# Dahan-Wang/Rethinking-Flow-and-Diffusion-Bridge-Models-for-Speech-Enhancement

Hardware: NVIDIA B200
Metric: enhanced audio-sec/sec (5-step SB bridge, ncsnpp_v2) (higher is better)
Workload: dtype fp16

## Files before the change

rethinking-flow-and-diffusion-bridge-models-for-speech-enhancement_b200/csrc/conv_igemm.cu:

```cuda
#include <cuda.h>
#include <mutex>
#include <type_traits>
#include "common.cuh"
#include "tc05.cuh"

namespace fdbm {
int make_act_tile_map(CUtensorMap* map, const op_t* ptr, int B, int T, int F, int C, int box_f, int box_t);
namespace {

using namespace tc05;

constexpr int MT = 2;
constexpr int TILE_T = 16, TILE_F = 8;
constexpr int HALO_T = TILE_T + 2, HALO_F = TILE_F + 2;
constexpr int A_TILE_BYTES = HALO_T * HALO_F * 128;
constexpr int A_TILE_STRIDE = 23552;
constexpr int A_STAGES = 3;
constexpr int B_STAGES = 3;
constexpr int BN = 128;
constexpr int B_TILE_BYTES = BN * 128;
constexpr int A_SBO = HALO_F * 128;
constexpr int NUM_THREADS = 512;
constexpr int EPI_GROUPS = 2;
constexpr int MAX_SEG = 3;
// ... 58 lines not shown

template <typename F>
__device__ __forceinline__ void walk_steps(const ConvParams& p, F&& f) {
  const int n_side = p.n_kb - p.n_main;
  int sd = 0, cnt = 0;
  for (int m = 0; m < p.n_main; ++m) {
    const int ntaps = p.seg[p.ksched[m] & 15].taps;
    for (int tap = 0; tap < ntaps; ++tap) {
      f(false, m, tap, ntaps);
      if (++cnt == p.side_gap && sd < n_side) { f(true, p.n_main + sd, 0, 1); ++sd; cnt = 0; }
    }
  }
  for (; sd < n_side; ++sd) f(true, p.n_main + sd, 0, 1);
}

template <bool COMB, bool RES16>
__global__ void __launch_bounds__(NUM_THREADS, 1)
conv_igemm_kernel(const __grid_constant__ CUtensorMap map_a0, const __grid_constant__ CUtensorMap map_a1,
                  const __grid_constant__ CUtensorMap map_a2, const __grid_constant__ CUtensorMap map_b,
                  const ConvParams p) {
  extern __shared__ __align__(1024) uint8_t smem_raw[];
  uint8_t* smem = smem_raw;
  if (smem_u32(smem_raw) & 1023u) __trap();
  uint8_t* sA = smem;
  uint8_t* sB = smem + A_STAGES * MT * A_TILE_STRIDE;
  uint8_t* s_stage = sB + B_STAGES * B_TILE_BYTES;
  uint8_t* s_stat = s_stage + STAGE_BYTES;
  uint64_t* bars = reinterpret_cast<uint64_t*>(s_stage + STAGE_BYTES + STAT_BYTES);
  uint64_t* a_full = bars;
  uint64_t* a_empty = a_full + A_STAGES;
  uint64_t* b_full = a_empty + A_STAGES;
  uint64_t* b_empty = b_full + B_STAGES_NARROW;
  uint64_t* acc_full = b_empty + B_STAGES_NARROW;
  const int b_stages = p.bn == 16 ? B_STAGES_NARROW : B_STAGES;
  const int b_stride = p.bn * 128;
  uint64_t* acc_empty = acc_full + 2;
  uint64_t* a_ready = acc_empty + 2;
  uint64_t* side_full = a_ready + A_STAGES;
  uint64_t* side_empty = side_full + 1;
  uint32_t* tmem_slot = reinterpret_cast<uint32_t*>(side_empty + 1);
  static_assert((3 * A_STAGES + 2 * B_STAGES_NARROW + 4 + 2) * 8 + 4 <= 512, "barrier region");
  const int a_stages = p.side_ring ? A_STAGES - 1 : A_STAGES;
  const int n_main = p.side_ring ? p.n_main : p.n_kb;

  const int warp = __shfl_sync(0xffffffffu, static_cast<int>(threadIdx.x >> 5), 0), lane = threadIdx.x & 31;
  const int n_kb = p.n_kb;

  if (threadIdx.x == 0) {
    for (int i = 0; i < A_STAGES; ++i) { mbar_init(a_full + i, 1); mbar_init(a_empty + i, 1); mbar_init(a_ready + i, 128); }
    for (int i = 0; i < B_STAGES_NARROW; ++i) { mbar_init(b_full + i, 1); mbar_init(b_empty + i, 1); }
    for (int i = 0; i < 2; ++i) { mbar_init(acc_full + i, 1); mbar_init(acc_empty + i, 4 * EPI_GROUPS); }
    mbar_init(side_full, 1); mbar_init(side_empty, 1);
    fence_barrier_init();
  }
  if (warp == 0 && lane == 0) {
    tma_prefetch_desc(&map_a0);
    tma_prefetch_desc(&map_b);
    if (p.n_seg > 1) tma_prefetch_desc(&map_a1);
    if (p.n_seg > 2) tma_prefetch_desc(&map_a2);
  }
  if (warp == 3) {
    tmem_alloc(tmem_slot, 512);
    tmem_relinquish();
  }
  fence_before_sync();
  __syncthreads();
  fence_after_sync();
  const uint32_t tmem_base = *tmem_slot;
  asm volatile("griddepcontrol.wait;" ::: "memory");
  asm volatile("griddepcontrol.launch_dependents;" ::: "memory");

  if (warp < 4) {
  reg_dec<PIPE_REGS>();
  if (warp == 0) {
    if (lane == 0) {
      uint32_t stage = 0, phase = 0;
      for (int item = blockIdx.x; item < p.n_items; item += gridDim.x) {
        const int ct = item_tile(p, item);
        TileCoord tc[MT];
        int n_valid = 0;
        for (int j = 0; j < MT; ++j) { tc[j] = decode_tile(p, ct * MT + j); n_valid += tc[j].valid; }
        for (int i = 0; i < n_main; ++i) {
          const uint32_t e = p.ksched[i];
          const int sgi = e & 15, c0 = ((e >> 4) & 0xFFF) * 64;
          const int halo = p.seg[sgi].halo;
          mbar_wait_relaxed<256>(a_empty + stage, phase ^ 1);
          mbar_expect_tx(a_full + stage, n_valid * (halo ? A_TILE_BYTES : A_TILE1_BYTES));
          const CUtensorMap* map = sgi == 0 ? &map_a0 : (sgi == 1 ? &map_a1 : &map_a2);
          for (int j = 0; j < MT; ++j) {
            if (!tc[j].valid) continue;
            tma_load_4d(sA + (stage * MT + j) * A_TILE_STRIDE, map, a_full + stage, c0, tc[j].f0 - halo, tc[j].t0 - halo,
                        tc[j].b);
          }
          if (++stage == a_stages) { stage = 0; phase ^= 1; }
        }
      }
    }
  } else if (warp == 3) {
    if (lane == 0 && p.side_ring) {
      uint32_t phase = 0;
      for (int item = blockIdx.x; item < p.n_items; item += gridDim.x) {
        const int ct = item_tile(p, item);
        TileCoord tc[MT];
        int n_valid = 0;
        for (int j = 0; j < MT; ++j) { tc[j] = decode_tile(p, ct * MT + j); n_valid += tc[j].valid; }
        for (int i = n_main; i < n_kb; ++i) {
          const uint32_t e = p.ksched[i];
          const int sgi = e & 15, c0 = ((e >> 4) & 0xFFF) * 64;
          mbar_wait_relaxed<128>(side_empty, phase ^ 1);
          mbar_expect_tx(side_full, n_valid * A_TILE1_BYTES);
          const CUtensorMap* map = sgi == 0 ? &map_a0 : (sgi == 1 ? &map_a1 : &map_a2);
          for (int j = 0; j < MT; ++j) {
            if (!tc[j].valid) continue;
            tma_load_4d(sA + ((A_STAGES - 1) * MT + j) * A_TILE_STRIDE, map, side_full, c0, tc[j].f0, tc[j].t0, tc[j].b);
          }
          phase ^= 1;
        }
      }
    }
  } else if (warp == 1) {
    if (lane == 0) {
      uint32_t stage = 0, phase = 0;
      for (int item = blockIdx.x; item < p.n_items; item += gridDim.x) {
        const int n0 = item_nblk(p, item) * BN;
        if (p.side_ring) {
          walk_steps(p, [&](bool, int idx, int tap, int) {
            const int kt = static_cast<int>(p.ksched[idx] >> 16) + tap;
            mbar_wait_relaxed<128>(b_empty + stage, phase ^ 1);
            mbar_expect_tx(b_full + stage, b_stride);
            tma_load_2d(sB + stage * b_stride, &map_b, b_full + stage, 0, kt * p.Cout + n0);
            if (++stage == b_stages) { stage = 0; phase ^= 1; }
          });
          continue;
        }
        for (int i = 0; i < n_kb; ++i) {
          const uint32_t e = p.ksched[i];
          const int ntaps = p.seg[e & 15].taps;
          int kt = e >> 16;
          for (int tap = 0; tap < ntaps; ++tap, ++kt) {
            mbar_wait_relaxed<128>(b_empty + stage, phase ^ 1);
            mbar_expect_tx(b_full + stage, b_stride);
            tma_load_2d(sB + stage * b_stride, &map_b, b_full + stage, 0, kt * p.Cout + n0);
            if (++stage == b_stages) { stage = 0; phase ^= 1; }
          }
        }
      }
    }
  } else if (warp == 2) {
    const uint32_t idesc = make_idesc_f16(128, p.bn, kOperandIsBf16);
    const uint64_t a_hi9 = make_desc_sw128(0, A_SBO) & 0xFFFFFFFF00000000ull;
    const uint64_t a_hi1 = make_desc_sw128(0, TILE_F * 128) & 0xFFFFFFFF00000000ull;
    const uint64_t b_hi = make_desc_sw128(0, 1024) & 0xFFFFFFFF00000000ull;
    const uint32_t lo_const = 1u << 16;
    const uint32_t sA_lo = (smem_u32(sA) & 0x3FFFF) >> 4, sB_lo = (smem_u32(sB) & 0x3FFFF) >> 4;
    uint32_t sa = 0, pa = 0, sb = 0, pb = 0, as = 0, pacc = 0, ps = 0;
    for (int item = blockIdx.x; item < p.n_items; item += gridDim.x) {
      const int ct = item_tile(p, item);
      const bool valid1 = (ct * MT + 1) < p.n_mtiles;
      mbar_wait(acc_empty + as, pacc ^ 1);
      fence_after_sync();
      uint32_t accumulate = 0;
      const uint32_t d0 = tmem_base + (as * MT) * BN, d1 = d0 + BN;
      if (p.side_ring) {
        int step = 0;
        walk_steps(p, [&](bool side, int idx, int tap, int ntaps) {
          const SegParams& sg = p.seg[p.ksched[idx] & 15];
          uint32_t a_base0, a_off = 0;
          if (side) {
            mbar_wait(side_full, ps);
            fence_after_sync();
            a_base0 = sA_lo + (((A_STAGES - 1) * MT) * A_TILE_STRIDE >> 4);
          } else {
            if (tap == 0) {
// ... 1 lines not shown
              fence_after_sync();
            }
            a_base0 = sA_lo + ((sa * MT) * A_TILE_STRIDE >> 4);
            const int df = ntaps == 9 ? tap / 3 : sg.halo, dt = ntaps == 9 ? tap - 3 * (tap / 3) : sg.halo;
            a_off = ((dt * HALO_F + df) * 128) >> 4;
          }
          const uint64_t a_hi = sg.halo ? a_hi9 : a_hi1;
          mbar_wait(b_full + sb, pb);
          fence_after_sync();
          const uint32_t b_lo = (sB_lo + (sb * b_stride >> 4)) | lo_const;
          const uint32_t a_lo0 = (a_base0 + a_off) | lo_const, a_lo1 = (a_base0 + (A_TILE_STRIDE >> 4) + a_off) | lo_const;
          const bool last_tap = tap == ntaps - 1;
          if (elect_one()) {
#pragma unroll
            for (int k = 0; k < 4; ++k)
              mma_f16(d0, a_hi | (a_lo0 + 2 * k), b_hi | (b_lo + 2 * k), idesc, k == 0 ? accumulate : 1u);
            if (valid1) {
#pragma unroll
              for (int k = 0; k < 4; ++k)
                mma_f16(d1, a_hi | (a_lo1 + 2 * k), b_hi | (b_lo + 2 * k), idesc, k == 0 ? accumulate : 1u);
            }
            mma_commit(b_empty + sb);
            if (side) mma_commit(side_empty);
            else if (last_tap) mma_commit(a_empty + sa);
            if (step == p.n_steps - 1) mma_commit(acc_full + as);
          }
          __syncwarp();
          accumulate = 1;
          ++step;
          if (++sb == b_stages) { sb = 0; pb ^= 1; }
          if (side) ps ^= 1;
          else if (last_tap && ++sa == a_stages) { sa = 0; pa ^= 1; }
        });
        if (++as == 2) { as = 0; pacc ^= 1; }
        continue;
      }
      for (int i = 0; i < n_kb; ++i) {
        const SegParams& sg = p.seg[p.ksched[i] & 15];
        const int ntaps = sg.taps;
        const uint64_t a_hi = sg.halo ? a_hi9 : a_hi1;
        mbar_wait(sg.norm ? a_ready + sa : a_full + sa, pa);
        fence_after_sync();
        const uint32_t a_base0 = sA_lo + ((sa * MT) * A_TILE_STRIDE >> 4), a_base1 = a_base0 + (A_TILE_STRIDE >> 4);
        int df = ntaps == 9 ? 0 : sg.halo, dt = df;
        for (int tap = 0; tap < ntaps; ++tap) {
          mbar_wait(b_full + sb, pb);
          fence_after_sync();
          const uint32_t a_off = ((dt * HALO_F + df) * 128) >> 4;
          const uint32_t b_lo = (sB_lo + (sb * b_stride >> 4)) | lo_const;
          const uint32_t a_lo0 = (a_base0 + a_off) | lo_const, a_lo1 = (a_base1 + a_off) | lo_const;
          if (elect_one()) {
#pragma unroll
            for (int k = 0; k < 4; ++k)
              mma_f16(d0, a_hi | (a_lo0 + 2 * k), b_hi | (b_lo + 2 * k), idesc, k == 0 ? accumulate : 1u);
            if (valid1) {
#pragma unroll
              for (int k = 0; k < 4; ++k)
                mma_f16(d1, a_hi | (a_lo1 + 2 * k), b_hi | (b_lo + 2 * k), idesc, k == 0 ? accumulate : 1u);
            }
            mma_commit(b_empty + sb);
            if (tap == ntaps - 1) mma_commit(a_empty + sa);
            if (tap == ntaps - 1 && i == n_kb - 1) mma_commit(acc_full + as);
          }
          __syncwarp();
          accumulate = 1;
          if (++dt == 3) { dt = 0; ++df; }
          if (++sb == b_stages) { sb = 0; pb ^= 1; }
        }
        if (++sa == A_STAGES) { sa = 0; pa ^= 1; }
      }
      if (++as == 2) { as = 0; pacc ^= 1; }
    }
  }
  } else if (warp >= 8 && warp < 12) {
    reg_dec<XFORM_REGS>();
    const int tt = threadIdx.x - 256;
    const int g = tt & 7, p_lane = tt >> 3;
    uint32_t stage = 0, phase = 0;
    const bool any_norm = (p.seg[0].norm | p.seg[1].norm | p.seg[2].norm) != 0;
    for (int item = blockIdx.x; any_norm && item < p.n_items; item += gridDim.x) {
      const int ct = item_tile(p, item);
      TileCoord tc[MT];
      for (int j = 0; j < MT; ++j) tc[j] = decode_tile(p, ct * MT + j);
      for (int i = 0; i < n_main; ++i) {
        const uint32_t e = p.ksched[i];
        const SegParams& sg = p.seg[e & 15];
        float2 sc[MT][4], sh[MT][4];
        if (sg.norm) {
          const int c0 = ((e >> 4) & 0xFFF) * 64 + g * 8;
          const float pre = sg.act ? 0.5f : 1.0f;
#pragma unroll
          for (int j = 0; j < MT; ++j) {
            const float4* tp = reinterpret_cast<const float4*>(sg.tab + static_cast<int64_t>(tc[j].valid ? tc[j].b : 0) * sg.tab_stride + c0);
#pragma unroll
            for (int u = 0; u < 4; ++u) {
              const float4 e = __ldg(tp + u);
              sc[j][u] = make_float2(pre * e.x, pre * e.z); sh[j][u] = make_float2(pre * e.y, pre * e.w);
            }
// ... 56 lines not shown
                  slot[u] = reinterpret_cast<uint4*>(tile + px * 128 + ((g ^ (px & 7)) << 4));
                  raw[u] = on[u] ? *slot[u] : make_uint4(0u, 0u, 0u, 0u);
                }
#pragma unroll
                for (int u = 0; u < 4; ++u) xform(raw[u], act_tag);
#pragma unroll
                for (int u = 0; u < 4; ++u)
                  if (on[u]) *slot[u] = raw[u];
              }
            };
            if (interior) { if (sg.act) run_interior(std::true_type{}); else run_interior(std::false_type{}); }
            else { if (sg.act) run_border(std::true_type{}); else run_border(std::false_type{}); }
          }
          fence_proxy_async();
        }
        mbar_arrive(a_ready + stage);
        if (++stage == a_stages) { stage = 0; phase ^= 1; }
      }
    }
  } else {
    reg_inc<EPI_REGS>();
    const int q = warp & 3;
    const int eg = warp >= 12 ? 1 : 0;
    float4* stage = reinterpret_cast<float4*>(s_stage) + (eg * 4 + q) * (32 * 8);
    const int cc = lane & 7;
    const int rsub = lane >> 3;
    const int et = (threadIdx.x & 127);
    uint32_t as = 0, pacc = 0;
    const bool do_stats = p.sums != nullptr;
    float2* wstat = reinterpret_cast<float2*>(s_stat) + eg * 4 * BN;
    double acc_s[STAT_SLOTS], acc_q[STAT_SLOTS];
// ... 1 lines not shown
    for (int u = 0; u < STAT_SLOTS; ++u) { acc_s[u] = 0.0; acc_q[u] = 0.0; }
    int stat_b = -1;
    auto flush_stats = [&]() {
#pragma unroll
      for (int u = 0; u < STAT_SLOTS; ++u) {
        if (u < p.n_nblocks) {
          if (et < p.bn) {
            double* dst = p.sums + (static_cast<int64_t>(stat_b) * p.Cout + u * BN + et) * 2;
            atomicAdd(dst, acc_s[u]);
            atomicAdd(dst + 1, acc_q[u]);
          }
        }
        acc_s[u] = 0.0; acc_q[u] = 0.0;
      }
    };
    for (int item = blockIdx.x; item < p.n_items; item += gridDim.x) {
      const int ct = item_tile(p, item);
      const int nblk = item - ct * p.n_nblocks;
      const int n0 = nblk * BN;
      mbar_wait_relaxed(acc_full + as, pacc);
      fence_after_sync();
      for (int j = eg; j <= eg; ++j) {
        const TileCoord tc = decode_tile(p, ct * MT + j);
        if (!tc.valid) continue;
        if (do_stats && stat_b != tc.b) {
          if (stat_b >= 0) flush_stats();
          stat_b = tc.b;
        }
        if (p.pyr_out) {
          uint32_t v[32];
          tmem_ld_32x32(tmem_base + ((q * 32u) << 16) + (as * MT + j) * BN, v);
          tmem_ld_wait();
          const int m = q * 32 + lane;
          const int t = tc.t0 + (m >> 3), f = tc.f0 + (m & 7);
          if (t < p.T && f < p.F) {
            float o[4];
#pragma unroll
            for (int c = 0; c < 4; ++c) o[c] = c < p.pyr_C ? __uint_as_float(v[c]) + __ldg(p.bias + c) : 0.f;
// ... 212 lines not shown
          __syncwarp();
          bv = bvn; bvb = bvbn;
        }
        if (do_stats) {
          asm volatile("bar.sync %0, 128;" ::"r"(1 + eg) : "memory");
          double s = 0.0, sq = 0.0;
#pragma unroll
          for (int w = 0; w < 4; ++w) { const float2 e = et < p.bn ? wstat[w * BN + et] : make_float2(0.f, 0.f); s += e.x; sq += e.y; }
#pragma unroll
          for (int u = 0; u < STAT_SLOTS; ++u) if (u == nblk) { acc_s[u] += s; acc_q[u] += sq; }
          asm volatile("bar.sync %0, 128;" ::"r"(1 + eg) : "memory");
        }
      }
      fence_before_sync();
      __syncwarp();
      if (lane == 0) mbar_arrive(acc_empty + as);
      if (++as == 2) { as = 0; pacc ^= 1; }
    }
    if (do_stats && stat_b >= 0) flush_stats();
  }

  fence_before_sync();
  __syncthreads();
  if (warp == 3) tmem_dealloc(tmem_base, 512);
}

__device__ __forceinline__ void pack_fwd_element(const PackDesc& d, int64_t i) {
  const int C1 = d.C1, C2 = d.C2, Cout = d.Cout, ksize = d.ksize, io_layout = d.io;
  const int taps = ksize * ksize;
  const int j = static_cast<int>(i % 64);
  const int co = static_cast<int>((i / 64) % Cout);
  const int kt = static_cast<int>(i / (64ll * Cout));
  float v;
  if (io_layout == 2) {
    const int tap = j / C1, ci = j % C1;
    v = tap < 9 ? d.w1[((static_cast<int64_t>(co) * C1 + ci) * 3 + tap / 3) * 3 + tap % 3] : 0.f;
  } else if (kt < (C1 / 64) * taps) {
    const int kb = kt / taps, tap = kt % taps;
    const int ci = kb * 64 + j;
// ... 66 lines not shown

int make_weight_map(CUtensorMap* map, const op_t* ptr, int64_t rows, int bn) {
  EncodeFn enc = get_encode();
  if (!enc) { set_error("cuTensorMapEncodeTiled entry point not available"); return FDBM_ECUDA; }
  cuuint64_t dims[2] = {64, (cuuint64_t)rows};
  cuuint64_t strides[1] = {128};
  cuuint32_t box[2] = {64, (cuuint32_t)bn};
  cuuint32_t es[2] = {1, 1};
  CUresult r = enc(map, (kOperandIsBf16 ? CU_TENSOR_MAP_DATA_TYPE_BFLOAT16 : CU_TENSOR_MAP_DATA_TYPE_FLOAT16), 2, const_cast<op_t*>(ptr), dims, strides, box, es,
                   CU_TENSOR_MAP_INTERLEAVE_NONE, CU_TENSOR_MAP_SWIZZLE_128B, CU_TENSOR_MAP_L2_PROMOTION_L2_256B,
                   CU_TENSOR_MAP_FLOAT_OOB_FILL_NONE);
  if (r != CUDA_SUCCESS) { set_error("cuTensorMapEncodeTiled(weights, %lld rows) failed: %d", (long long)rows, (int)r); return FDBM_ECUDA; }
  return FDBM_OK;
}

}

int make_act_tile_map(CUtensorMap* map, const op_t* ptr, int B, int T, int F, int C, int box_f, int box_t) {
  EncodeFn enc = get_encode();
  if (!enc) { set_error("cuTensorMapEncodeTiled entry point not available"); return FDBM_ECUDA; }
  cuuint64_t dims[4] = {(cuuint64_t)C, (cuuint64_t)F, (cuuint64_t)T, (cuuint64_t)B};
  cuuint64_t strides[3] = {(cuuint64_t)C * 2, (cuuint64_t)C * 2 * F, (cuuint64_t)C * 2 * F * T};
  cuuint32_t box[4] = {64, (cuuint32_t)box_f, (cuuint32_t)box_t, 1};
  cuuint32_t es[4] = {1, 1, 1, 1};
  CUresult r = enc(map, (kOperandIsBf16 ? CU_TENSOR_MAP_DATA_TYPE_BFLOAT16 : CU_TENSOR_MAP_DATA_TYPE_FLOAT16), 4, const_cast<op_t*>(ptr), dims, strides, box, es,
                   CU_TENSOR_MAP_INTERLEAVE_NONE, CU_TENSOR_MAP_SWIZZLE_128B, CU_TENSOR_MAP_L2_PROMOTION_L2_256B,
                   CU_TENSOR_MAP_FLOAT_OOB_FILL_NONE);
  if (r != CUDA_SUCCESS) { set_error("cuTensorMapEncodeTiled(activation [%d,%d,%d,%d]) failed: %d", B, T, F, C, (int)r); return FDBM_ECUDA; }
  return FDBM_OK;
}
// ... 49 lines not shown
  const PackDesc d = pack_desc_dgrad(w, Cout, Cin, ksize, wpack, Cin_total, ci_off);
  pack_one_kernel<<<static_cast<int>(std::min<int64_t>(ceil_div64(d.total, 256), 4096)), 256, 0, s>>>(d);
  FDBM_LAUNCH_CHECK();
  return FDBM_OK;
}

int launch_conv_igemm(const ConvArgs& a, cudaStream_t s) {
  FDBM_REQUIRE(a.n_seg >= 1 && a.n_seg <= MAX_SEG, "conv_igemm: 1..%d K segments", MAX_SEG);
  const int bn = a.narrow_n ? 16 : (a.Cout == 64 ? 64 : BN);
  FDBM_REQUIRE(a.Cout % bn == 0 && (!a.narrow_n || (a.Cout == 16 && a.pyr_out)), "conv_igemm: Cout must be a multiple of %d (got %d)", bn, a.Cout);
  FDBM_REQUIRE(a.out_f32 || a.out_h16 || a.pyr_out, "conv_igemm: no output");
  FDBM_REQUIRE(!a.pyr_out || (a.pyr_C >= 1 && a.pyr_C <= 4 && a.Cout == bn && !a.sums), "conv_igemm: bad pyramid epilogue arguments");
  FDBM_REQUIRE(!a.pyr_prev || (a.T % 2 == 0 && a.F % 2 == 0), "conv_igemm: pyramid level with odd size");
  static PerDeviceOnce attr_once;
  if (attr_once.first(current_device())) {
    FDBM_CUDA(cudaFuncSetAttribute(conv_igemm_kernel<false, false>, cudaFuncAttributeMaxDynamicSharedMemorySize, SMEM_BYTES));
    FDBM_CUDA(cudaFuncSetAttribute(conv_igemm_kernel<false, true>, cudaFuncAttributeMaxDynamicSharedMemorySize, SMEM_BYTES));
    FDBM_CUDA(cudaFuncSetAttribute(conv_igemm_kernel<true, false>, cudaFuncAttributeMaxDynamicSharedMemorySize, SMEM_BYTES));
  }
  FDBM_REQUIRE(!a.comb_pyr || (a.comb_w && a.comb_b && a.comb_C >= 1 && a.comb_C <= 4 && !a.pyr_out), "conv_igemm: bad Combine epilogue arguments");
  CUtensorMap map_a[MAX_SEG], map_b;
  ConvParams p;
  p.B = a.B; p.T = a.T; p.F = a.F; p.Cout = a.Cout;
  p.n_seg = a.n_seg;
  int kb = 0, n_kt = 0;
  for (int i = 0; i < MAX_SEG; ++i) {
    if (i < a.n_seg) {
      const ConvSeg& sg = a.seg[i];
      FDBM_REQUIRE(sg.in && sg.C > 0 && sg.C % 64 == 0 && (sg.taps == 9 || sg.taps == 1),
                   "conv_igemm: segment %d needs a tensor, C %% 64 == 0 and 9 or 1 taps (C=%d, taps=%d)", i, sg.C, sg.taps);
      const int halo = sg.taps == 9 || sg.norm_tab != nullptr;
      if (int rc = halo ? make_act_map(&map_a[i], sg.in, a.B, a.T, a.F, sg.C)
                        : make_act_tile_map(&map_a[i], sg.in, a.B, a.T, a.F, sg.C, TILE_F, TILE_T)) return rc;
// ... 17 lines not shown
        const uint32_t e = static_cast<uint32_t>(i) | (static_cast<uint32_t>(cb) << 4) | (static_cast<uint32_t>(kt) << 16);
        if (a.seg[i].taps == 9) nine[n9++] = e; else one[n1++] = e;
        kt += a.seg[i].taps;
      }
    int n = 0;
    for (int i = 0; i < n9; ++i) p.ksched[n++] = nine[i];
    for (int i = 0; i < n1; ++i) p.ksched[n++] = one[i];
    for (; n < MAX_KB; ++n) p.ksched[n] = 0;
    bool side_ok = n1 > 0 && n9 > 0;
    for (int i = 0; i < a.n_seg; ++i) side_ok = side_ok && (a.seg[i].taps == 9 || !p.seg[i].halo);
    p.side_ring = side_ok ? 1 : 0;
    p.n_main = p.side_ring ? n9 : kb;
    p.side_gap = p.side_ring ? std::max(3, ceil_div(9 * n9, n1)) : 0;
    p.n_steps = n_kt;
  }
  if (int rc = make_weight_map(&map_b, a.wpack, static_cast<int64_t>(n_kt) * a.Cout, bn)) return rc;
  p.bn = bn;
  p.tiles_t = ceil_div(a.T, TILE_T); p.tiles_f = ceil_div(a.F, TILE_F);
  p.n_mtiles = a.B * p.tiles_t * p.tiles_f;
  p.n_nblocks = a.Cout / bn;
  p.n_items = ceil_div(p.n_mtiles, MT) * p.n_nblocks;
  {
    auto magic = [](int d) { return static_cast<uint32_t>((0x100000000ull + d - 1) / static_cast<uint64_t>(d)); };
    p.mg_tiles_t = magic(p.tiles_t); p.mg_tiles_f = magic(p.tiles_f); p.mg_nblocks = magic(p.n_nblocks);
    const int64_t dmax = std::max(std::max(p.tiles_t, p.tiles_f), p.n_nblocks);
    FDBM_REQUIRE((2 * (static_cast<int64_t>(p.n_items) + num_sms()) + 2) * dmax < 0x100000000ll, "conv_igemm: %d items exceed the range of the index arithmetic", p.n_items);
  }
  p.bias = a.bias; p.bias_b = a.bias_b; p.bias_b_stride = a.bias_b_stride; p.residual = a.residual; p.scale = a.scale;
  p.residual_h16 = a.residual_h16;
  FDBM_REQUIRE(!(a.residual && a.residual_h16) && !(a.residual_h16 && (a.comb_pyr || a.pyr_out)), "conv_igemm: bad residual arguments");
  p.out_f32 = a.out_f32; p.out_h16 = a.out_h16; p.sums = a.sums;
  p.pyr_out = a.pyr_out; p.pyr_prev = a.pyr_prev; p.pyr_C = a.pyr_C;
  p.comb_pyr = a.comb_pyr; p.comb_w = a.comb_w; p.comb_b = a.comb_b; p.comb_C = a.comb_C;
  if (a.sums) {
    FDBM_REQUIRE(p.n_nblocks <= STAT_SLOTS, "conv_igemm: channel sums support Cout <= %d", STAT_SLOTS * BN);
    if (!a.sums_prezeroed) FDBM_CUDA(cudaMemsetAsync(a.sums, 0, sizeof(double) * 2 * a.B * a.Cout, s));
  }
  const int grid = std::min(p.n_items, num_sms());
  cudaLaunchConfig_t cfg = {};
  cfg.gridDim = dim3(grid); cfg.blockDim = dim3(NUM_THREADS); cfg.dynamicSmemBytes = SMEM_BYTES; cfg.stream = s;
  cudaLaunchAttribute attr[1];
  attr[0].id = cudaLaunchAttributeProgrammaticStreamSerialization;
  attr[0].val.programmaticStreamSerializationAllowed = 1;
  cfg.attrs = attr; cfg.numAttrs = pdl_enabled() && a.B <= pdl_batch_limit() ? 1 : 0;
  if (a.comb_pyr) FDBM_CUDA(cudaLaunchKernelEx(&cfg, conv_igemm_kernel<true, false>, map_a[0], map_a[1], map_a[2], map_b, p));
  else if (a.residual_h16) FDBM_CUDA(cudaLaunchKernelEx(&cfg, conv_igemm_kernel<false, true>, map_a[0], map_a[1], map_a[2], map_b, p));
  else FDBM_CUDA(cudaLaunchKernelEx(&cfg, conv_igemm_kernel<false, false>, map_a[0], map_a[1], map_a[2], map_b, p));
  FDBM_LAUNCH_CHECK();
  return FDBM_OK;
}

}

using namespace fdbm;

extern "C" int fdbm_pack_conv_weights(const float* w1, int C1, int ksize, const float* w2, int C2, int Cout,
                                      void* wpack, int64_t* bytes, void* stream) {
  const int k = ksize == -1 ? 1 : ksize;
  if (bytes) *bytes = ksize == -2 ? static_cast<int64_t>(Cout) * 64 * 2 : conv_wpack_bytes(C1, k, C2, Cout);
  if (!wpack) return FDBM_OK;
  if (int rc = require_sm100()) return rc;
  FDBM_REQUIRE(w1 && ((C2 == 0) == (w2 == nullptr)), "fdbm_pack_conv_weights: null pointer");
// ... 55 lines not shown
```

rethinking-flow-and-diffusion-bridge-models-for-speech-enhancement_b200/csrc/tc05.cuh:

```cuda
#pragma once
#include <cuda.h>
#include <cuda_runtime.h>
#include <stdint.h>

namespace tc05 {

__device__ __forceinline__ uint32_t smem_u32(const void* p) {
  return static_cast<uint32_t>(__cvta_generic_to_shared(p));
}

__device__ __forceinline__ bool elect_one() {
  uint32_t pred = 0;
  asm volatile(
      "{\n\t.reg .pred P;\n\t"
      "elect.sync _|P, 0xffffffff;\n\t"
      "selp.u32 %0, 1, 0, P;\n\t}\n"
      : "=r"(pred));
  return pred != 0;
}

#if 0
template <int N> __device__ __forceinline__ void reg_dec() {}
template <int N> __device__ __forceinline__ void reg_inc() {}
#else
// ... 86 lines not shown
  asm volatile("tcgen05.fence::after_thread_sync;" ::: "memory");
}
__device__ __forceinline__ void mma_f16(uint32_t tmem_d, uint64_t desc_a, uint64_t desc_b, uint32_t idesc,
                                         uint32_t accumulate) {
  asm volatile(
      "{\n\t.reg .pred p;\n\t"
      "setp.ne.b32 p, %4, 0;\n\t"
      "tcgen05.mma.cta_group::1.kind::f16 [%0], %1, %2, %3, p;\n\t}\n"
      ::"r"(tmem_d), "l"(desc_a), "l"(desc_b), "r"(idesc), "r"(accumulate)
      : "memory");
}
__device__ __forceinline__ void mma_commit(uint64_t* bar) {
  asm volatile("tcgen05.commit.cta_group::1.mbarrier::arrive::one.shared::cluster.b64 [%0];" ::"r"(smem_u32(bar))
               : "memory");
}
__device__ __forceinline__ void tmem_ld_32x32(uint32_t taddr, uint32_t (&r)[32]) {
  asm volatile(
      "tcgen05.ld.sync.aligned.32x32b.x32.b32 "
      "{%0, %1, %2, %3, %4, %5, %6, %7, %8, %9, %10, %11, %12, %13, %14, %15, "
      "%16, %17, %18, %19, %20, %21, %22, %23, %24, %25, %26, %27, %28, %29, %30, %31}, [%32];"
      : "=r"(r[0]), "=r"(r[1]), "=r"(r[2]), "=r"(r[3]), "=r"(r[4]), "=r"(r[5]), "=r"(r[6]), "=r"(r[7]),
        "=r"(r[8]), "=r"(r[9]), "=r"(r[10]), "=r"(r[11]), "=r"(r[12]), "=r"(r[13]), "=r"(r[14]), "=r"(r[15]),
        "=r"(r[16]), "=r"(r[17]), "=r"(r[18]), "=r"(r[19]), "=r"(r[20]), "=r"(r[21]), "=r"(r[22]), "=r"(r[23]),
        "=r"(r[24]), "=r"(r[25]), "=r"(r[26]), "=r"(r[27]), "=r"(r[28]), "=r"(r[29]), "=r"(r[30]), "=r"(r[31])
      : "r"(taddr)
      : "memory");
}
__device__ __forceinline__ void tmem_ld_wait() { asm volatile("tcgen05.wait::ld.sync.aligned;" ::: "memory"); }

__device__ __forceinline__ uint64_t make_desc_sw128(uint32_t smem_addr, uint32_t sbo_bytes, uint32_t base_offset = 0) {
// ... 18 lines not shown
```

Baseline: 1318.

## Add paired-CTA (cta_group::2) path for conv implicit-GEMM with split weight tiles

Result: faster. 1353, median of 6 (+2.7%).

```diff
diff --git a/rethinking-flow-and-diffusion-bridge-models-for-speech-enhancement_b200/csrc/conv_igemm.cu b/rethinking-flow-and-diffusion-bridge-models-for-speech-enhancement_b200/csrc/conv_igemm.cu
--- a/rethinking-flow-and-diffusion-bridge-models-for-speech-enhancement_b200/csrc/conv_igemm.cu
+++ b/rethinking-flow-and-diffusion-bridge-models-for-speech-enhancement_b200/csrc/conv_igemm.cu
@@ -96,11 +96,26 @@
   for (; sd < n_side; ++sd) f(true, p.n_main + sd, 0, 1);
 }
 
-template <bool COMB, bool RES16>
+template <bool PAIR> __device__ __forceinline__ bool is_leader() { return !PAIR || (blockIdx.x & 1) == 0; }
+template <bool PAIR> __device__ __forceinline__ int first_item() {
+  return PAIR ? static_cast<int>((blockIdx.x >> 1) + (blockIdx.x & 1) * (gridDim.x >> 1)) : static_cast<int>(blockIdx.x);
+}
+template <bool PAIR> __device__ __forceinline__ bool walk_on(const ConvParams& p, int item) {
+  return (PAIR ? item - static_cast<int>((blockIdx.x & 1) * (gridDim.x >> 1)) : item) < p.n_items;
+}
+__device__ __forceinline__ int valid_tiles(const ConvParams& p, int item) {
+  int n = 0;
+  if (item < p.n_items)
+    for (int j = 0; j < MT; ++j) n += decode_tile(p, item_tile(p, item) * MT + j).valid;
+  return n;
+}
+
+template <bool COMB, bool RES16, bool PAIR>
 __global__ void __launch_bounds__(NUM_THREADS, 1)
 conv_igemm_kernel(const __grid_constant__ CUtensorMap map_a0, const __grid_constant__ CUtensorMap map_a1,
                   const __grid_constant__ CUtensorMap map_a2, const __grid_constant__ CUtensorMap map_b,
                   const ConvParams p) {
+  static_assert(!(PAIR && COMB), "the Combine epilogue has no paired instantiation");
   extern __shared__ __align__(1024) uint8_t smem_raw[];
   uint8_t* smem = smem_raw;
   if (smem_u32(smem_raw) & 1023u) __trap();
@@ -114,8 +129,8 @@
   uint64_t* b_full = a_empty + A_STAGES;
   uint64_t* b_empty = b_full + B_STAGES_NARROW;
   uint64_t* acc_full = b_empty + B_STAGES_NARROW;
-  const int b_stages = p.bn == 16 ? B_STAGES_NARROW : B_STAGES;
-  const int b_stride = p.bn * 128;
+  const int b_stages = p.bn == 16 ? B_STAGES_NARROW : (PAIR ? 2 * B_STAGES : B_STAGES);
+  const int b_stride = PAIR ? B_TILE_BYTES / 2 : p.bn * 128;
   uint64_t* acc_empty = acc_full + 2;
   uint64_t* a_ready = acc_empty + 2;
   uint64_t* side_full = a_ready + A_STAGES;
@@ -129,9 +144,9 @@
   const int n_kb = p.n_kb;
 
   if (threadIdx.x == 0) {
-    for (int i = 0; i < A_STAGES; ++i) { mbar_init(a_full + i, 1); mbar_init(a_empty + i, 1); mbar_init(a_ready + i, 128); }
+    for (int i = 0; i < A_STAGES; ++i) { mbar_init(a_full + i, 1); mbar_init(a_empty + i, 1); mbar_init(a_ready + i, PAIR ? 8 : 128); }
     for (int i = 0; i < B_STAGES_NARROW; ++i) { mbar_init(b_full + i, 1); mbar_init(b_empty + i, 1); }
-    for (int i = 0; i < 2; ++i) { mbar_init(acc_full + i, 1); mbar_init(acc_empty + i, 4 * EPI_GROUPS); }
+    for (int i = 0; i < 2; ++i) { mbar_init(acc_full + i, 1); mbar_init(acc_empty + i, 4 * EPI_GROUPS * (PAIR ? 2 : 1)); }
     mbar_init(side_full, 1); mbar_init(side_empty, 1);
     fence_barrier_init();
   }
@@ -141,14 +156,16 @@
     if (p.n_seg > 1) tma_prefetch_desc(&map_a1);
     if (p.n_seg > 2) tma_prefetch_desc(&map_a2);
   }
+  if (PAIR) cluster_barrier_sync();
   if (warp == 3) {
-    tmem_alloc(tmem_slot, 512);
-    tmem_relinquish();
+    if (PAIR) { tmem_alloc_pair(tmem_slot, 512); tmem_relinquish_pair(); }
+    else { tmem_alloc(tmem_slot, 512); tmem_relinquish(); }
   }
   fence_before_sync();
   __syncthreads();
   fence_after_sync();
   const uint32_t tmem_base = *tmem_slot;
+  if (PAIR) cluster_barrier_sync();
   asm volatile("griddepcontrol.wait;" ::: "memory");
   asm volatile("griddepcontrol.launch_dependents;" ::: "memory");
 
@@ -157,60 +174,90 @@
   if (warp == 0) {
     if (lane == 0) {
       uint32_t stage = 0, phase = 0;
-      for (int item = blockIdx.x; item < p.n_items; item += gridDim.x) {
+      const uint32_t a_full_leader = PAIR ? mapa_shared(smem_u32(a_full), 0) : 0u;
+      for (int item = first_item<PAIR>(); walk_on<PAIR>(p, item); item += gridDim.x) {
         const int ct = item_tile(p, item);
         TileCoord tc[MT];
         int n_valid = 0;
-        for (int j = 0; j < MT; ++j) { tc[j] = decode_tile(p, ct * MT + j); n_valid += tc[j].valid; }
+        for (int j = 0; j < MT; ++j) { tc[j] = decode_tile(p, item < p.n_items ? ct * MT + j : p.n_mtiles); n_valid += tc[j].valid; }
+        const int n_valid_peer = PAIR && is_leader<PAIR>() ? valid_tiles(p, item + (gridDim.x >> 1)) : 0;
         for (int i = 0; i < n_main; ++i) {
           const uint32_t e = p.ksched[i];
           const int sgi = e & 15, c0 = ((e >> 4) & 0xFFF) * 64;
           const int halo = p.seg[sgi].halo;
+          const int tile_bytes = halo ? A_TILE_BYTES : A_TILE1_BYTES;
+          const bool via_leader = PAIR && !p.seg[sgi].norm;
           mbar_wait_relaxed<256>(a_empty + stage, phase ^ 1);
-          mbar_expect_tx(a_full + stage, n_valid * (halo ? A_TILE_BYTES : A_TILE1_BYTES));
+          if (!via_leader) mbar_expect_tx(a_full + stage, n_valid * tile_bytes);
+          else if (is_leader<PAIR>()) mbar_expect_tx(a_full + stage, (n_valid + n_valid_peer) * tile_bytes);
           const CUtensorMap* map = sgi == 0 ? &map_a0 : (sgi == 1 ? &map_a1 : &map_a2);
           for (int j = 0; j < MT; ++j) {
             if (!tc[j].valid) continue;
-            tma_load_4d(sA + (stage * MT + j) * A_TILE_STRIDE, map, a_full + stage, c0, tc[j].f0 - halo, tc[j].t0 - halo,
-                        tc[j].b);
+            void* dst = sA + (stage * MT + j) * A_TILE_STRIDE;
+            if (via_leader && !is_leader<PAIR>())
+              tma_load_4d_pair(dst, map, a_full_leader + stage * 8, c0, tc[j].f0 - halo, tc[j].t0 - halo, tc[j].b);
+            else
+              tma_load_4d(dst, map, a_full + stage, c0, tc[j].f0 - halo, tc[j].t0 - halo, tc[j].b);
           }
           if (++stage == a_stages) { stage = 0; phase ^= 1; }
         }
+      }
+      for (int i = 0; PAIR && i < a_stages; ++i) {
+        mbar_wait_relaxed<256>(a_empty + stage, phase ^ 1);
+        if (++stage == a_stages) { stage = 0; phase ^= 1; }
       }
     }
   } else if (warp == 3) {
     if (lane == 0 && p.side_ring) {
       uint32_t phase = 0;
-      for (int item = blockIdx.x; item < p.n_items; item += gridDim.x) {
+      const uint32_t side_full_leader = PAIR ? mapa_shared(smem_u32(side_full), 0) : 0u;
+      for (int item = first_item<PAIR>(); walk_on<PAIR>(p, item); item += gridDim.x) {
         const int ct = item_tile(p, item);
         TileCoord tc[MT];
         int n_valid = 0;
-        for (int j = 0; j < MT; ++j) { tc[j] = decode_tile(p, ct * MT + j); n_valid += tc[j].valid; }
+        for (int j = 0; j < MT; ++j) { tc[j] = decode_tile(p, item < p.n_items ? ct * MT + j : p.n_mtiles); n_valid += tc[j].valid; }
+        const int n_valid_peer = PAIR && is_leader<PAIR>() ? valid_tiles(p, item + (gridDim.x >> 1)) : 0;
         for (int i = n_main; i < n_kb; ++i) {
           const uint32_t e = p.ksched[i];
           const int sgi = e & 15, c0 = ((e >> 4) & 0xFFF) * 64;
           mbar_wait_relaxed<128>(side_empty, phase ^ 1);
-          mbar_expect_tx(side_full, n_valid * A_TILE1_BYTES);
+          if (is_leader<PAIR>()) mbar_expect_tx(side_full, (n_valid + n_valid_peer) * A_TILE1_BYTES);
           const CUtensorMap* map = sgi == 0 ? &map_a0 : (sgi == 1 ? &map_a1 : &map_a2);
           for (int j = 0; j < MT; ++j) {
             if (!tc[j].valid) continue;
-            tma_load_4d(sA + ((A_STAGES - 1) * MT + j) * A_TILE_STRIDE, map, side_full, c0, tc[j].f0, tc[j].t0, tc[j].b);
+            void* dst = sA + ((A_STAGES - 1) * MT + j) * A_TILE_STRIDE;
+            if (PAIR && !is_leader<PAIR>()) tma_load_4d_pair(dst, map, side_full_leader, c0, tc[j].f0, tc[j].t0, tc[j].b);
+            else tma_load_4d(dst, map, side_full, c0, tc[j].f0, tc[j].t0, tc[j].b);
           }
           phase ^= 1;
         }
       }
+      if (PAIR) mbar_wait_relaxed<128>(side_empty, phase ^ 1);
     }
   } else if (warp == 1) {
     if (lane == 0) {
       uint32_t stage = 0, phase = 0;
-      for (int item = blockIdx.x; item < p.n_items; item += gridDim.x) {
+      const uint32_t b_full_leader = PAIR ? mapa_shared(smem_u32(b_full), 0) : 0u;
+      auto fetch = [&](uint32_t stage, int kt, int n0) {
+        if (PAIR) {
+          if (is_leader<PAIR>()) {
+            mbar_expect_tx(b_full + stage, B_TILE_BYTES);
+            tma_load_2d(sB + stage * b_stride, &map_b, b_full + stage, 0, kt * p.Cout + n0);
+          } else {
+            tma_load_2d_pair(sB + stage * b_stride, &map_b, b_full_leader + stage * 8, 0, kt * p.Cout + n0 + BN / 2);
+          }
+        } else {
+          mbar_expect_tx(b_full + stage, b_stride);
+          tma_load_2d(sB + stage * b_stride, &map_b, b_full + stage, 0, kt * p.Cout + n0);
+        }
+      };
+      for (int item = first_item<PAIR>(); walk_on<PAIR>(p, item); item += gridDim.x) {
         const int n0 = item_nblk(p, item) * BN;
         if (p.side_ring) {
           walk_steps(p, [&](bool, int idx, int tap, int) {
             const int kt = static_cast<int>(p.ksched[idx] >> 16) + tap;
             mbar_wait_relaxed<128>(b_empty + stage, phase ^ 1);
-            mbar_expect_tx(b_full + stage, b_stride);
-            tma_load_2d(sB + stage * b_stride, &map_b, b_full + stage, 0, kt * p.Cout + n0);
+            fetch(stage, kt, n0);
             if (++stage == b_stages) { stage = 0; phase ^= 1; }
           });
           continue;
@@ -221,24 +268,31 @@
           int kt = e >> 16;
           for (int tap = 0; tap < ntaps; ++tap, ++kt) {
             mbar_wait_relaxed<128>(b_empty + stage, phase ^ 1);
-            mbar_expect_tx(b_full + stage, b_stride);
-            tma_load_2d(sB + stage * b_stride, &map_b, b_full + stage, 0, kt * p.Cout + n0);
+            fetch(stage, kt, n0);
             if (++stage == b_stages) { stage = 0; phase ^= 1; }
           }
         }
+      }
+      for (int i = 0; PAIR && i < b_stages; ++i) {
+        mbar_wait_relaxed<128>(b_empty + stage, phase ^ 1);
+        if (++stage == b_stages) { stage = 0; phase ^= 1; }
       }
     }
   } else if (warp == 2) {
-    const uint32_t idesc = make_idesc_f16(128, p.bn, kOperandIsBf16);
+    const uint32_t idesc = make_idesc_f16(PAIR ? 256 : 128, p.bn, kOperandIsBf16);
     const uint64_t a_hi9 = make_desc_sw128(0, A_SBO) & 0xFFFFFFFF00000000ull;
     const uint64_t a_hi1 = make_desc_sw128(0, TILE_F * 128) & 0xFFFFFFFF00000000ull;
     const uint64_t b_hi = make_desc_sw128(0, 1024) & 0xFFFFFFFF00000000ull;
     const uint32_t lo_const = 1u << 16;
     const uint32_t sA_lo = (smem_u32(sA) & 0x3FFFF) >> 4, sB_lo = (smem_u32(sB) & 0x3FFFF) >> 4;
     uint32_t sa = 0, pa = 0, sb = 0, pb = 0, as = 0, pacc = 0, ps = 0;
-    for (int item = blockIdx.x; item < p.n_items; item += gridDim.x) {
+    auto mma = [&](uint32_t d, uint64_t da, uint64_t db, uint32_t acc) {
+      if (PAIR) mma_f16_pair(d, da, db, idesc, acc); else mma_f16(d, da, db, idesc, acc);
+    };
+    auto commit = [&](uint64_t* bar) { if (PAIR) mma_commit_pair(bar); else mma_commit(bar); };
+    for (int item = first_item<PAIR>(); item < p.n_items && is_leader<PAIR>(); item += gridDim.x) {
       const int ct = item_tile(p, item);
-      const bool valid1 = (ct * MT + 1) < p.n_mtiles;
+      const bool valid1 = PAIR || (ct * MT + 1) < p.n_mtiles;
       mbar_wait(acc_empty + as, pacc ^ 1);
       fence_after_sync();
       uint32_t accumulate = 0;
@@ -270,16 +324,16 @@
           if (elect_one()) {
 #pragma unroll
             for (int k = 0; k < 4; ++k)
-              mma_f16(d0, a_hi | (a_lo0 + 2 * k), b_hi | (b_lo + 2 * k), idesc, k == 0 ? accumulate : 1u);
+              mma(d0, a_hi | (a_lo0 + 2 * k), b_hi | (b_lo + 2 * k), k == 0 ? accumulate : 1u);
             if (valid1) {
 #pragma unroll
               for (int k = 0; k < 4; ++k)
-                mma_f16(d1, a_hi | (a_lo1 + 2 * k), b_hi | (b_lo + 2 * k), idesc, k == 0 ? accumulate : 1u);
-            }
-            mma_commit(b_empty + sb);
-            if (side) mma_commit(side_empty);
-            else if (last_tap) mma_commit(a_empty + sa);
-            if (step == p.n_steps - 1) mma_commit(acc_full + as);
+                mma(d1, a_hi | (a_lo1 + 2 * k), b_hi | (b_lo + 2 * k), k == 0 ? accumulate : 1u);
+            }
+            commit(b_empty + sb);
+            if (side) commit(side_empty);
+            else if (last_tap) commit(a_empty + sa);
+            if (step == p.n_steps - 1) commit(acc_full + as);
           }
           __syncwarp();
           accumulate = 1;
@@ -308,15 +362,15 @@
           if (elect_one()) {
 #pragma unroll
             for (int k = 0; k < 4; ++k)
-              mma_f16(d0, a_hi | (a_lo0 + 2 * k), b_hi | (b_lo + 2 * k), idesc, k == 0 ? accumulate : 1u);
+              mma(d0, a_hi | (a_lo0 + 2 * k), b_hi | (b_lo + 2 * k), k == 0 ? accumulate : 1u);
             if (valid1) {
 #pragma unroll
               for (int k = 0; k < 4; ++k)
-                mma_f16(d1, a_hi | (a_lo1 + 2 * k), b_hi | (b_lo + 2 * k), idesc, k == 0 ? accumulate : 1u);
-            }
-            mma_commit(b_empty + sb);
-            if (tap == ntaps - 1) mma_commit(a_empty + sa);
-            if (tap == ntaps - 1 && i == n_kb - 1) mma_commit(acc_full + as);
+                mma(d1, a_hi | (a_lo1 + 2 * k), b_hi | (b_lo + 2 * k), k == 0 ? accumulate : 1u);
+            }
+            commit(b_empty + sb);
+            if (tap == ntaps - 1) commit(a_empty + sa);
+            if (tap == ntaps - 1 && i == n_kb - 1) commit(acc_full + as);
           }
           __syncwarp();
           accumulate = 1;
@@ -334,10 +388,10 @@
     const int g = tt & 7, p_lane = tt >> 3;
     uint32_t stage = 0, phase = 0;
     const bool any_norm = (p.seg[0].norm | p.seg[1].norm | p.seg[2].norm) != 0;
-    for (int item = blockIdx.x; any_norm && item < p.n_items; item += gridDim.x) {
+    for (int item = first_item<PAIR>(); any_norm && walk_on<PAIR>(p, item); item += gridDim.x) {
       const int ct = item_tile(p, item);
       TileCoord tc[MT];
-      for (int j = 0; j < MT; ++j) tc[j] = decode_tile(p, ct * MT + j);
+      for (int j = 0; j < MT; ++j) tc[j] = decode_tile(p, item < p.n_items ? ct * MT + j : p.n_mtiles);
       for (int i = 0; i < n_main; ++i) {
         const uint32_t e = p.ksched[i];
         const SegParams& sg = p.seg[e & 15];
@@ -424,7 +478,12 @@
           }
           fence_proxy_async();
         }
-        mbar_arrive(a_ready + stage);
+        if (PAIR) {
+          __syncwarp();
+          if (lane == 0) mbar_arrive_cluster(mapa_shared(smem_u32(a_ready + stage), 0));
+        } else {
+          mbar_arrive(a_ready + stage);
+        }
         if (++stage == a_stages) { stage = 0; phase ^= 1; }
       }
     }
@@ -456,14 +515,15 @@
         acc_s[u] = 0.0; acc_q[u] = 0.0;
       }
     };
-    for (int item = blockIdx.x; item < p.n_items; item += gridDim.x) {
+    const uint32_t acc_empty_leader = PAIR ? mapa_shared(smem_u32(acc_empty), 0) : 0u;
+    for (int item = first_item<PAIR>(); walk_on<PAIR>(p, item); item += gridDim.x) {
       const int ct = item_tile(p, item);
       const int nblk = item - ct * p.n_nblocks;
       const int n0 = nblk * BN;
       mbar_wait_relaxed(acc_full + as, pacc);
       fence_after_sync();
       for (int j = eg; j <= eg; ++j) {
-        const TileCoord tc = decode_tile(p, ct * MT + j);
+        const TileCoord tc = decode_tile(p, item < p.n_items ? ct * MT + j : p.n_mtiles);
         if (!tc.valid) continue;
         if (do_stats && stat_b != tc.b) {
           if (stat_b >= 0) flush_stats();
@@ -706,7 +766,7 @@
       }
       fence_before_sync();
       __syncwarp();
-      if (lane == 0) mbar_arrive(acc_empty + as);
+      if (lane == 0) { if (PAIR) mbar_arrive_cluster(acc_empty_leader + as * 8); else mbar_arrive(acc_empty + as); }
       if (++as == 2) { as = 0; pacc ^= 1; }
     }
     if (do_stats && stat_b >= 0) flush_stats();
@@ -714,7 +774,8 @@
 
   fence_before_sync();
   __syncthreads();
-  if (warp == 3) tmem_dealloc(tmem_base, 512);
+  if (PAIR) cluster_barrier_sync();
+  if (warp == 3) { if (PAIR) tmem_dealloc_pair(tmem_base, 512); else tmem_dealloc(tmem_base, 512); }
 }
 
 __device__ __forceinline__ void pack_fwd_element(const PackDesc& d, int64_t i) {
@@ -811,6 +872,35 @@
   return FDBM_OK;
 }
 
+int pair_grid(int* out) {
+  static int cached[64] = {};
+  const int dev = current_device();
+  if (dev >= 0 && dev < 64 && cached[dev]) { *out = cached[dev]; return FDBM_OK; }
+  cudaLaunchConfig_t cfg = {};
+  cfg.gridDim = dim3(num_sms() & ~1); cfg.blockDim = dim3(NUM_THREADS); cfg.dynamicSmemBytes = SMEM_BYTES;
+  cudaLaunchAttribute attr;
+  attr.id = cudaLaunchAttributeClusterDimension;
+  attr.val.clusterDim.x = 2; attr.val.clusterDim.y = 1; attr.val.clusterDim.z = 1;
+  cfg.attrs = &attr; cfg.numAttrs = 1;
+  int n = 0;
+  FDBM_CUDA(cudaOccupancyMaxActiveClusters(&n, conv_igemm_kernel<false, false, true>, &cfg));
+  *out = std::min(2 * n, num_sms() & ~1);
+  if (dev >= 0 && dev < 64) cached[dev] = *out;
+  return FDBM_OK;
+}
+
+bool conv_pair_rule(const ConvParams& p, bool pyr_epilogue, int pair_grid, int* grid) {
+  if (p.bn != BN || pyr_epilogue || pair_grid < 2 || p.n_items < 2 * pair_grid || (pair_grid / 2) % p.n_nblocks != 0) return false;
+  int n9 = 0;
+  for (int i = 0; i < p.n_seg; ++i) n9 += p.seg[i].taps == 9;
+  if (n9 != 1) return false;
+  const int main_end = p.side_ring ? p.n_main : p.n_kb;
+  for (int i = 1; i < main_end; ++i)
+    if (p.seg[p.ksched[i] & 15].norm != p.seg[p.ksched[0] & 15].norm) return false;
+  *grid = pair_grid;
+  return true;
+}
+
 }
 
 int make_act_tile_map(CUtensorMap* map, const op_t* ptr, int B, int T, int F, int C, int box_f, int box_t) {
@@ -890,9 +980,11 @@
   FDBM_REQUIRE(!a.pyr_prev || (a.T % 2 == 0 && a.F % 2 == 0), "conv_igemm: pyramid level with odd size");
   static PerDeviceOnce attr_once;
   if (attr_once.first(current_device())) {
-    FDBM_CUDA(cudaFuncSetAttribute(conv_igemm_kernel<false, false>, cudaFuncAttributeMaxDynamicSharedMemorySize, SMEM_BYTES));
-    FDBM_CUDA(cudaFuncSetAttribute(conv_igemm_kernel<false, true>, cudaFuncAttributeMaxDynamicSharedMemorySize, SMEM_BYTES));
-    FDBM_CUDA(cudaFuncSetAttribute(conv_igemm_kernel<true, false>, cudaFuncAttributeMaxDynamicSharedMemorySize, SMEM_BYTES));
+    FDBM_CUDA(cudaFuncSetAttribute(conv_igemm_kernel<false, false, false>, cudaFuncAttributeMaxDynamicSharedMemorySize, SMEM_BYTES));
+    FDBM_CUDA(cudaFuncSetAttribute(conv_igemm_kernel<false, true, false>, cudaFuncAttributeMaxDynamicSharedMemorySize, SMEM_BYTES));
+    FDBM_CUDA(cudaFuncSetAttribute(conv_igemm_kernel<true, false, false>, cudaFuncAttributeMaxDynamicSharedMemorySize, SMEM_BYTES));
+    FDBM_CUDA(cudaFuncSetAttribute(conv_igemm_kernel<false, false, true>, cudaFuncAttributeMaxDynamicSharedMemorySize, SMEM_BYTES));
+    FDBM_CUDA(cudaFuncSetAttribute(conv_igemm_kernel<false, true, true>, cudaFuncAttributeMaxDynamicSharedMemorySize, SMEM_BYTES));
   }
   FDBM_REQUIRE(!a.comb_pyr || (a.comb_w && a.comb_b && a.comb_C >= 1 && a.comb_C <= 4 && !a.pyr_out), "conv_igemm: bad Combine epilogue arguments");
   CUtensorMap map_a[MAX_SEG], map_b;
@@ -940,7 +1032,6 @@
     p.side_gap = p.side_ring ? std::max(3, ceil_div(9 * n9, n1)) : 0;
     p.n_steps = n_kt;
   }
-  if (int rc = make_weight_map(&map_b, a.wpack, static_cast<int64_t>(n_kt) * a.Cout, bn)) return rc;
   p.bn = bn;
   p.tiles_t = ceil_div(a.T, TILE_T); p.tiles_f = ceil_div(a.F, TILE_F);
   p.n_mtiles = a.B * p.tiles_t * p.tiles_f;
@@ -962,16 +1053,30 @@
     FDBM_REQUIRE(p.n_nblocks <= STAT_SLOTS, "conv_igemm: channel sums support Cout <= %d", STAT_SLOTS * BN);
     if (!a.sums_prezeroed) FDBM_CUDA(cudaMemsetAsync(a.sums, 0, sizeof(double) * 2 * a.B * a.Cout, s));
   }
-  const int grid = std::min(p.n_items, num_sms());
+  int grid = std::min(p.n_items, num_sms()), grid2 = 0;
+  if (int rc = pair_grid(&grid2)) return rc;
+  const bool pair = conv_pair_rule(p, a.comb_pyr != nullptr || a.pyr_out != nullptr, grid2, &grid);
+  if (int rc = make_weight_map(&map_b, a.wpack, static_cast<int64_t>(n_kt) * a.Cout, pair ? bn / 2 : bn)) return rc;
   cudaLaunchConfig_t cfg = {};
   cfg.gridDim = dim3(grid); cfg.blockDim = dim3(NUM_THREADS); cfg.dynamicSmemBytes = SMEM_BYTES; cfg.stream = s;
-  cudaLaunchAttribute attr[1];
-  attr[0].id = cudaLaunchAttributeProgrammaticStreamSerialization;
-  attr[0].val.programmaticStreamSerializationAllowed = 1;
-  cfg.attrs = attr; cfg.numAttrs = pdl_enabled() && a.B <= pdl_batch_limit() ? 1 : 0;
-  if (a.comb_pyr) FDBM_CUDA(cudaLaunchKernelEx(&cfg, conv_igemm_kernel<true, false>, map_a[0], map_a[1], map_a[2], map_b, p));
-  else if (a.residual_h16) FDBM_CUDA(cudaLaunchKernelEx(&cfg, conv_igemm_kernel<false, true>, map_a[0], map_a[1], map_a[2], map_b, p));
-  else FDBM_CUDA(cudaLaunchKernelEx(&cfg, conv_igemm_kernel<false, false>, map_a[0], map_a[1], map_a[2], map_b, p));
+  cudaLaunchAttribute attr[2];
+  int n_attr = 0;
+  if (pdl_enabled() && a.B <= pdl_batch_limit()) {
+    attr[n_attr].id = cudaLaunchAttributeProgrammaticStreamSerialization;
+    attr[n_attr].val.programmaticStreamSerializationAllowed = 1;
+    ++n_attr;
+  }
+  if (pair) {
+    attr[n_attr].id = cudaLaunchAttributeClusterDimension;
+    attr[n_attr].val.clusterDim.x = 2; attr[n_attr].val.clusterDim.y = 1; attr[n_attr].val.clusterDim.z = 1;
+    ++n_attr;
+  }
+  cfg.attrs = attr; cfg.numAttrs = n_attr;
+  if (a.comb_pyr) FDBM_CUDA(cudaLaunchKernelEx(&cfg, conv_igemm_kernel<true, false, false>, map_a[0], map_a[1], map_a[2], map_b, p));
+  else if (a.residual_h16 && pair) FDBM_CUDA(cudaLaunchKernelEx(&cfg, conv_igemm_kernel<false, true, true>, map_a[0], map_a[1], map_a[2], map_b, p));
+  else if (a.residual_h16) FDBM_CUDA(cudaLaunchKernelEx(&cfg, conv_igemm_kernel<false, true, false>, map_a[0], map_a[1], map_a[2], map_b, p));
+  else if (pair) FDBM_CUDA(cudaLaunchKernelEx(&cfg, conv_igemm_kernel<false, false, true>, map_a[0], map_a[1], map_a[2], map_b, p));
+  else FDBM_CUDA(cudaLaunchKernelEx(&cfg, conv_igemm_kernel<false, false, false>, map_a[0], map_a[1], map_a[2], map_b, p));
   FDBM_LAUNCH_CHECK();
   return FDBM_OK;
 }
diff --git a/rethinking-flow-and-diffusion-bridge-models-for-speech-enhancement_b200/csrc/tc05.cuh b/rethinking-flow-and-diffusion-bridge-models-for-speech-enhancement_b200/csrc/tc05.cuh
--- a/rethinking-flow-and-diffusion-bridge-models-for-speech-enhancement_b200/csrc/tc05.cuh
+++ b/rethinking-flow-and-diffusion-bridge-models-for-speech-enhancement_b200/csrc/tc05.cuh
@@ -124,6 +124,50 @@
   asm volatile("tcgen05.commit.cta_group::1.mbarrier::arrive::one.shared::cluster.b64 [%0];" ::"r"(smem_u32(bar))
                : "memory");
 }
+__device__ __forceinline__ uint32_t mapa_shared(uint32_t local_addr, uint32_t rank) {
+  uint32_t r; asm volatile("mapa.shared::cluster.u32 %0, %1, %2;" : "=r"(r) : "r"(local_addr), "r"(rank)); return r;
+}
+__device__ __forceinline__ void cluster_barrier_sync() {
+  asm volatile("barrier.cluster.arrive.release;" ::: "memory");
+  asm volatile("barrier.cluster.wait.acquire;" ::: "memory");
+}
+__device__ __forceinline__ void mbar_arrive_cluster(uint32_t bar_cluster_addr) {
+  asm volatile("mbarrier.arrive.release.cluster.shared::cluster.b64 _, [%0];" ::"r"(bar_cluster_addr) : "memory");
+}
+__device__ __forceinline__ void tmem_alloc_pair(uint32_t* dst_smem, uint32_t ncols) {
+  asm volatile("tcgen05.alloc.cta_group::2.sync.aligned.shared::cta.b32 [%0], %1;" ::"r"(smem_u32(dst_smem)), "r"(ncols) : "memory");
+}
+__device__ __forceinline__ void tmem_relinquish_pair() { asm volatile("tcgen05.relinquish_alloc_permit.cta_group::2.sync.aligned;" ::: "memory"); }
+__device__ __forceinline__ void tmem_dealloc_pair(uint32_t addr, uint32_t ncols) {
+  asm volatile("tcgen05.dealloc.cta_group::2.sync.aligned.b32 %0, %1;" ::"r"(addr), "r"(ncols) : "memory");
+}
+__device__ __forceinline__ void mma_f16_pair(uint32_t tmem_d, uint64_t desc_a, uint64_t desc_b, uint32_t idesc, uint32_t accumulate) {
+  asm volatile(
+      "{\n\t.reg .pred p;\n\t"
+      "setp.ne.b32 p, %4, 0;\n\t"
+      "tcgen05.mma.cta_group::2.kind::f16 [%0], %1, %2, %3, p;\n\t}\n"
+      ::"r"(tmem_d), "l"(desc_a), "l"(desc_b), "r"(idesc), "r"(accumulate)
+      : "memory");
+}
+__device__ __forceinline__ void mma_commit_pair(uint64_t* bar) {
+  const uint16_t mask = 3;
+  asm volatile("tcgen05.commit.cta_group::2.mbarrier::arrive::one.shared::cluster.multicast::cluster.b64 [%0], %1;" ::"r"(smem_u32(bar)), "h"(mask)
+               : "memory");
+}
+__device__ __forceinline__ void tma_load_2d_pair(void* dst, const CUtensorMap* m, uint32_t bar_cluster_addr, int c0, int c1) {
+  asm volatile(
+      "cp.async.bulk.tensor.2d.cta_group::2.shared::cluster.global.mbarrier::complete_tx::bytes [%0], [%1, {%3, %4}], [%2];"
+      ::"r"(smem_u32(dst)), "l"(reinterpret_cast<uint64_t>(m)), "r"(bar_cluster_addr), "r"(c0), "r"(c1)
+      : "memory");
+}
+__device__ __forceinline__ void tma_load_4d_pair(void* dst, const CUtensorMap* m, uint32_t bar_cluster_addr, int c0, int c1, int c2,
+                                                 int c3) {
+  asm volatile(
+      "cp.async.bulk.tensor.4d.cta_group::2.shared::cluster.global.mbarrier::complete_tx::bytes [%0], [%1, {%3, %4, %5, %6}], [%2];"
+      ::"r"(smem_u32(dst)), "l"(reinterpret_cast<uint64_t>(m)), "r"(bar_cluster_addr), "r"(c0), "r"(c1), "r"(c2), "r"(c3)
+      : "memory");
+}
+
 __device__ __forceinline__ void tmem_ld_32x32(uint32_t taddr, uint32_t (&r)[32]) {
   asm volatile(
       "tcgen05.ld.sync.aligned.32x32b.x32.b32 "
```
